# mschoenb97/po2_quantization

Measured on AMD Instinct MI355X. Metric: quantized-conv fwd images/sec, ResNet56 224×224 bs=256; 1/2/4/8 MI355X, higher is better.
Workload: dtype fp32(bf16x3); 1 GPU; resnet56 quantized-conv chain: 56 fused po2-4bit quantize+conv fwd + head (stage-1 and stage-2 conv1->conv2 pairs as one launch each) (stride-2 conv1 + 1x1 shortcut of stages 2-3 as one launch each) (weight packs of the single-conv layers batched: one launch per 36); conv_pairs=True, conv_pairs_stage2=True, s2ds=True, pack_batch=True, autotune=True, image=224, batch_per_gpu=256, global_batch=256, quantizer=po2, bits=4, precision=bf16x3, parallelism=dp1, world_size=1, hip_graph=False

## Files before the change

### po2_quantization_amd/csrc/po2q_capi.hip

```cpp
#include <hip/hip_runtime.h>

#include <cstdio>
#include <algorithm>
#include <new>
#include <cstring>
#include <string>
#include <vector>

#include "../../include/po2q.h"
#include "po2q_epi.h"
#include "po2q_internal.h"

namespace po2q {
static thread_local std::string g_last_error;
void set_error(const std::string& msg) { g_last_error = msg; }
}

using namespace po2q;

namespace {

constexpr size_t kAlign = 256;
size_t align_up(size_t v) { return (v + kAlign - 1) / kAlign * kAlign; }

// ... 875 lines not shown

int po2q_qconv2d_ir_f32(const float* x, float* y, const po2q_conv_plan* expand, const void* ws_e, size_t ws_e_bytes,
                        const po2q_conv_plan* depthwise, const void* ws_d, size_t ws_d_bytes,
                        const po2q_conv_plan* project, const void* ws_p, size_t ws_p_bytes, const float* ps1,
                        const float* pb1, int act1, const float* ps2, const float* pb2, int act2, const float* ps3,
                        const float* pb3, const float* residual, int act3, void* stream) {
    using namespace po2q;
    if (!x || !y || !ws_d || !ws_p || (expand && !ws_e)) {
        set_error("po2q: inverted residual: null pointer");
        return PO2Q_ERR_INVALID;
    }
    for (int a : {act1, act2, act3})
        if (a < PO2Q_ACT_NONE || a > PO2Q_ACT_SILU) {
            set_error("po2q: unknown activation " + std::to_string(a));
            return PO2Q_ERR_INVALID;
        }
    IrPlan ip;
    int64_t sh[7];
    int st = ir_check(expand, depthwise, project, &ip, sh);
    if (st) return st;
    const po2q_conv_plan* hs[3] = {expand, depthwise, project};
    const void* wss[3] = {ws_e, ws_d, ws_p};
    const size_t wsb[3] = {ws_e_bytes, ws_d_bytes, ws_p_bytes};
    const char* at[3] = {nullptr, nullptr, nullptr};
    const float* sc[3] = {nullptr, nullptr, nullptr};
    for (int i = 0; i < 3; ++i) {
        if (!hs[i]) continue;
        const WsLayout L = ws_layout(hs[i]->p, hs[i]->mode);
        if (wsb[i] < L.total) {
            set_error("po2q: inverted residual: workspace too small (need " + std::to_string(L.total) + " bytes)");
            return PO2Q_ERR_WORKSPACE;
        }
        at[i] = reinterpret_cast<const char*>(wss[i]) + L.packed_off;
        sc[i] = reinterpret_cast<const float*>(reinterpret_cast<const char*>(wss[i]) + L.scale_off);
    }
    const IrEpi ep{ps1, pb1, ps2, pb2, ps3, pb3, act1, act2, act3, residual};
    return hip_status(launch_conv_ir(ip, x, y, (int)sh[0], (int)sh[1], (int)sh[2], (int)sh[3], (int)sh[4], (int)sh[5],
                                     (int)sh[6], reinterpret_cast<const uint16_t*>(at[0]), sc[0],
                                     reinterpret_cast<const float*>(at[1]), reinterpret_cast<const uint16_t*>(at[2]),
                                     sc[2], ep, reinterpret_cast<hipStream_t>(stream)),
                      "inverted residual launch");
}

int po2q_qconv2d_plan_describe(const po2q_conv_plan* plan, char* buf, size_t len) {
    if (!plan || !buf || len == 0) {
        po2q::set_error("po2q: null plan or buffer");
        return PO2Q_ERR_INVALID;
    }
    describe_plan(plan->p, buf, len);
    return PO2Q_OK;
}

void po2q_qconv2d_plan_destroy(po2q_conv_plan* plan) { delete plan; }
```

### po2_quantization_amd/csrc/po2q_conv_chain.hip

```cpp
#include <hip/hip_runtime.h>

#include <algorithm>
#include <cstddef>
#include <cstdint>
#include <cstdlib>
#include <string>
#include <type_traits>
#include <utility>
#include <vector>

#include "../../include/po2q.h"
#ifdef PO2Q_CHAIN_STAMPS
#include <cstdio>
#endif
#include "po2q_epi.h"
#include "po2q_internal.h"
#include "po2q_x3_dev.h"

namespace po2q {

namespace {
constexpr int kChainThreads = 512;
constexpr int kChainItems = 5;
constexpr int kChainMax = PO2Q_CHAIN_MAX_LAYERS;
// ... 367 lines not shown
#endif
}

static int chain_mg(int64_t C, int64_t H, int64_t W) {
    const int64_t groups = (H * W + 15) / 16, wpt = (kChainThreads / 64) / (C / 16);
    return (int)((groups + wpt - 1) / wpt);
}
static int chain_mg_max(int64_t C) { return C == 16 ? 8 : 4; }

static bool chain_geom_ok(int64_t N, int64_t C, int64_t H, int64_t W, int n_layers) {
    if (!(C == 16 || C == 32 || C == 64) || N < 1 || H < 1 || W < 4 || W % 4 != 0) return false;
    if (n_layers < 1 || n_layers > kChainMax || N > INT32_MAX) return false;
    if (N * C * H * W >= (1LL << 40) || chain_mg(C, H, W) > chain_mg_max(C)) return false;
    return 3 * chain_plane(C, H, W) <= kChainLdsMax;
}

static bool chain_mode_ok(int bits, int fsr, int mode) {
    if (mode != PO2Q_MODE_PO2 && mode != PO2Q_MODE_PO2_PLUS) return false;
    if (bits < 1 || bits > 16) return false;
    const long lo = (long)fsr - (1L << (bits - 1)), hi = (long)fsr - 1;
    return lo >= -126 && hi <= 127;
}

static ConvPlan chain_plan(int64_t N, int64_t C, int64_t H, int64_t W) {
    ConvPlan p{};
    p.N = (int)N; p.C = (int)C; p.H = (int)H; p.W = (int)W; p.K = (int)C;
    p.R = p.S = 3; p.sh = p.sw = 1; p.ph = p.pw = 1; p.dh = p.dw = 1; p.groups = 1;
    p.P = p.H; p.Q = p.W; p.Cg = p.C; p.Kg = p.K;
    p.kind = KIND_BF16X3_IMG;
    p.CC = C == 16 ? 16 : 32;
    p.nchunks = (int)C / p.CC;
    p.steps = C == 16 ? 2 : 3 * p.nchunks;
    p.NT = (int)C / 16;
    p.taps = 9;
    p.packed_floats = (int64_t)3 * p.steps * p.NT * 64 * 4;
    return p;
}

namespace {
constexpr size_t kChainAlign = 256;
size_t chain_align(size_t v) { return (v + kChainAlign - 1) / kChainAlign * kChainAlign; }
struct ChainWs {
    size_t packed_off, packed_bytes, scale_off, total;
};
ChainWs chain_ws(int64_t N, int64_t C, int64_t H, int64_t W, int n_layers) {
    ChainWs L;
    const ConvPlan p = chain_plan(N, C, H, W);
    L.packed_bytes = chain_align((size_t)p.packed_floats * 4);
    L.packed_off = 0;
    L.scale_off = L.packed_bytes * (size_t)n_layers;
    L.total = L.scale_off + chain_align((size_t)n_layers * 4);
    return L;
}
}

}

using namespace po2q;

extern "C" {

int po2q_qconv2d_chain_supported(int64_t N, int64_t C, int64_t H, int64_t W, int n_layers, int bits, int fsr,
                                 int mode) {
    return chain_geom_ok(N, C, H, W, n_layers) && chain_mode_ok(bits, fsr, mode) ? 1 : 0;
}

size_t po2q_qconv2d_chain_workspace_bytes(int64_t N, int64_t C, int64_t H, int64_t W, int n_layers) {
    if (!chain_geom_ok(N, C, H, W, n_layers)) return 0;
    return chain_ws(N, C, H, W, n_layers).total;
}

int po2q_qconv2d_chain_f32(const float* x, const float* const* w, const float* const* bias,
                           const float* const* post_scale, const float* const* post_shift, const int* act,
                           const int* res_from, int n_layers, int64_t N, int64_t C, int64_t H, int64_t W, int bits,
                           int fsr, int mode, float* y, void* workspace, size_t workspace_bytes, void* stream) {
    if (po2q::is_lin_mode(mode)) {
        po2q::set_error("po2q: chain does not take the lin / lin+ modes");
        return PO2Q_ERR_UNSUPPORTED;
    }
    if (!chain_geom_ok(N, C, H, W, n_layers)) {
        set_error("po2q: chain needs C in {16, 32, 64}, W % 4 == 0, 1.." + std::to_string(kChainMax) +
                  " layers and a small image: its split planes in LDS ((H + 2)(W + 2) 6C bytes <= 160 KiB) and "
                  "at most 8 (C = 16) / 4 (C = 32, 64) 16-pixel groups per wave");
        return PO2Q_ERR_INVALID;
    }
    if (!chain_mode_ok(bits, fsr, mode)) {
        set_error("po2q: chain needs mode po2 / po2+ with exponents in the bf16 range");
        return PO2Q_ERR_INVALID;
    }
    if (!x || !w || !y || !workspace) {
        set_error("po2q: chain: null pointer");
        return PO2Q_ERR_INVALID;
    }
    const ChainWs L = chain_ws(N, C, H, W, n_layers);
    if (workspace_bytes < L.total) {
        set_error("po2q: chain workspace too small (need " + std::to_string(L.total) + " bytes)");
        return PO2Q_ERR_WORKSPACE;
    }
    for (int l = 0; l < n_layers; ++l) {
        if (!w[l]) {
            set_error("po2q: chain: null weight of layer " + std::to_string(l));
            return PO2Q_ERR_INVALID;
        }
        const int ac = act ? act[l] : 0;
        if (ac < 0 || ac > 3) {
            set_error("po2q: chain: unknown activation of layer " + std::to_string(l));
            return PO2Q_ERR_INVALID;
        }
        const int r = res_from ? res_from[l] : -1;
        if (r < -1 || r > l) {
            set_error("po2q: chain: res_from[" + std::to_string(l) + "] must be -1 or a layer index <= " +
                      std::to_string(l) + " (the residual is that layer's input)");
            return PO2Q_ERR_INVALID;
        }
    }
    for (int l1 = 0; l1 < n_layers; ++l1)
        for (int l2 = l1 + 1; l2 < n_layers; ++l2) {
            const int r1 = res_from ? res_from[l1] : -1, r2 = res_from ? res_from[l2] : -1;
            if (r1 >= 0 && r2 >= 0 && r1 != r2 && r2 <= l1) {
                set_error("po2q: chain: res_from holds one residual source at a time (layers " + std::to_string(l1) +
                          " and " + std::to_string(l2) + " add different, overlapping sources)");
                return PO2Q_ERR_INVALID;
            }
        }
    hipStream_t s = reinterpret_cast<hipStream_t>(stream);
    char* ws = reinterpret_cast<char*>(workspace);

    const ConvPlan plan = chain_plan(N, C, H, W);
    std::vector<const ConvPlan*> plans((size_t)n_layers, &plan);
    std::vector<uint16_t*> packed((size_t)n_layers);
    std::vector<float*> scales((size_t)n_layers);
    for (int l = 0; l < n_layers; ++l) {
        packed[l] = reinterpret_cast<uint16_t*>(ws + L.packed_off + (size_t)l * L.packed_bytes);
        scales[l] = reinterpret_cast<float*>(ws + L.scale_off) + l;
    }
    hipError_t he = launch_pack_bf16x3_batch(n_layers, plans.data(), w, packed.data(), scales.data(), bits, fsr,
                                             mode, s);
    if (he != hipSuccess) {
        set_error(std::string("po2q: chain weight pack launch: ") + hipGetErrorString(he));
        return PO2Q_ERR_HIP;
    }

    std::vector<int> used((size_t)n_layers + 1, 0);
    for (int l = 0; l < n_layers; ++l)
        if (res_from && res_from[l] >= 0) used[res_from[l]] = 1;
    ChainArgs a{};
    a.stamps = nullptr;
    a.H = (int)H; a.W = (int)W; a.L = n_layers;
    a.PW = (int)W + 2;
    a.PL = (int)chain_plane(C, H, W);
    a.ZO = a.PL - 16;
    a.res0 = used[0];
    for (int l = 0; l < n_layers; ++l) {
        ChainLayer& ly = a.layer[l];
        ly.wp = reinterpret_cast<const uint4*>(packed[l]);
        ly.scale = scales[l];
        ly.bias = bias ? bias[l] : nullptr;
        ly.ps = post_scale ? post_scale[l] : nullptr;
        ly.pb = post_shift ? post_shift[l] : nullptr;
        ly.act = act ? act[l] : 0;
        ly.res_add = (res_from && res_from[l] >= 0) ? 1 : 0;
        ly.keep = used[l + 1];
    }
    const char* venv = getenv("PO2Q_CHAIN_VARIANT");
    const int variant = venv ? atoi(venv) : 0;
    const bool db = !(variant & 8) && C != 16 && 6 * (size_t)a.PL <= kChainLdsMax;
    const size_t lds = (db ? 6 : 3) * (size_t)a.PL;
    const dim3 grid((unsigned)N), block(kChainThreads);
    const int mg = chain_mg(C, H, W);
    const bool w8 = C == 64 && W == 8;
    const int64_t wpt = (kChainThreads / 64) / (C / 16);
    const bool full = !(variant & 1) && (H * W) % 16 == 0 && (H * W / 16) % wpt == 0;
    auto launch = [&](const ChainArgs& a) -> bool {
#define PO2Q_CH(c, m, w)                                                                               \
    if (C == c && mg <= m && w8 == w) {                                                                \
        if (c != 16 && db) {                                                                           \
            if (full && mg == m)                                                                       \
                hipLaunchKernelGGL((conv_chain<c, m, w, true, true>), grid, block, lds, s, x, y, a);   \
            else                                                                                       \
// ... 52 lines not shown
```

### po2_quantization_amd/csrc/po2q_conv_pair.hip

```cpp
#include <hip/hip_runtime.h>

#include <algorithm>
#include <climits>
#include <cstdint>
#include <string>
#include <type_traits>
#ifdef PO2Q_PAIR_STAMPS
#include <cstdio>
#include <cstdlib>
#include <vector>
#endif

#include "../../include/po2q.h"
#include "po2q_epi.h"
#include "po2q_internal.h"
#include "po2q_quant_dev.h"
#include "po2q_rows_dev.h"
#include "po2q_x3_dev.h"

namespace po2q {

namespace {
template <int CC> constexpr int kQSW = 512 / CC;
template <int CC> constexpr int kQPlane = (kQSW<CC> + 2) * 2 * CC + 32;
// ... 1004 lines not shown
        return pp.pd == 3 ? launch_pair_rs<3>(pp, a, x, y, s) : hipErrorInvalidValue;
    }
#ifdef PO2Q_PAIR_DIAG
    if (const char* dv = getenv("PO2Q_PAIR_DEBUG")) {
        const int dbg = atoi(dv);
        const dim3 grid((unsigned)pp.blocks), block(64 * pp.waves);
#define PO2Q_PD(v) \
        if (dbg == v && pp.C == 16 && pp.pd == 2 && pp.nts == 3 && !res) { \
            hipLaunchKernelGGL((conv_pair<16, 2, 3, false, 0, v>), grid, block, pp.lds, s, x, y, a); \
            return hipGetLastError(); \
        }
        PO2Q_PD(1) PO2Q_PD(2) PO2Q_PD(3) PO2Q_PD(4) PO2Q_PD(8) PO2Q_PD(12) PO2Q_PD(16) PO2Q_PD(19)
        PO2Q_PD(15) PO2Q_PD(31)
#undef PO2Q_PD
    }
#endif
#define PO2Q_PR(c, d, nt) \
    if (pp.C == c && pp.pd == d && pp.nts == nt) return launch_pair_t<c, d, nt>(pp, a, x, y, res, s);
#ifdef PO2Q_PAIR_ISA_ONLY
    PO2Q_PR(16, 5, 3) PO2Q_PR(32, 2, 3)
    return hipErrorInvalidValue;
#endif
    PO2Q_PR(16, 2, 0) PO2Q_PR(16, 2, 1) PO2Q_PR(16, 2, 3) PO2Q_PR(32, 2, 0) PO2Q_PR(32, 2, 3)
    PO2Q_PR(16, 5, 3) PO2Q_PR(16, 6, 3)
#undef PO2Q_PR
    return hipErrorInvalidValue;
}

}

namespace {

void pair_variant(int& pd, int& nts, int& prio, int64_t C) {
    pd = 2;
    nts = 3;
    prio = C == 16 ? 1 : 0;
    if (const char* e = getenv("PO2Q_PAIR_VARIANT")) {
        const int v = atoi(e) % 1000;
        const int d = (v / 10) % 10, t = v % 10;
        prio = v >= 100 ? 1 : 0;
        if (d == 2 && (t == 0 || t == 3 || (t == 1 && C == 16))) {
            pd = d;
            nts = t;
        }
    }
}

bool pair_args_ok(int64_t N, int64_t C, int64_t H, int64_t W, int bits, int fsr, int mode, int act1, int act2) {
    if (N <= 0 || H <= 0 || W <= 0) {
        po2q::set_error("po2q: pair: sizes must be positive");
        return false;
    }
    if (C != 16 && C != 32) {
        po2q::set_error("po2q: pair: 16 or 32 channels only (ResNet56 stages 1 and 2)");
        return false;
    }
    if (mode != PO2Q_MODE_PO2 && mode != PO2Q_MODE_PO2_PLUS) {
        po2q::set_error("po2q: pair: mode must be po2 or po2+");
        return false;
    }
    if (bits < 1 || bits > 16) {
        po2q::set_error("po2q: bits must be in [1, 16]");
        return false;
    }
    const long lo = (long)fsr - (1L << (bits - 1)), hi = (long)fsr - 1;
    if (lo < -126 || hi > 127) {
        po2q::set_error("po2q: pair: the exponent window leaves the bf16 range");
        return false;
    }
    if (act1 < 0 || act1 > 3 || act2 < 0 || act2 > 3) {
        po2q::set_error("po2q: unknown activation");
        return false;
    }
    if (W % 4 != 0 || W > 7 * (512 / C)) {
        po2q::set_error("po2q: pair: W must be a multiple of 4 and at most 7 x 512 / C (224 for C = 16, 112 for 32)");
        return false;
    }
    return true;
}

}

int po2q_qconv2d_pair_supported(int64_t N, int64_t C, int64_t H, int64_t W, int bits, int fsr, int mode) {
    if ((C == 16 || C == 32) && W <= 3 * (512 / C)) return 0;
    if (C == 32) {
        const char* e = getenv("PO2Q_PAIR_C32");
        if (e && e[0] == '0') return 0;
    }
    po2q::PairPlan pp;
    int pd, nts, prio;
    pair_variant(pd, nts, prio, C);
    return pair_args_ok(N, C, H, W, bits, fsr, mode, 0, 0) &&
                   po2q::pair_plan(pp, (int)N, (int)C, (int)H, (int)W, true, pd, nts)
               ? 1
               : 0;
}

int po2q_qconv2d_pair_f32(const float* x, const float* w1, const float* w2, float* y, int64_t N, int64_t C,
                          int64_t H, int64_t W, int bits, int fsr, int mode, const float* bias1, const float* bias2,
                          const float* post_scale1, const float* post_shift1, int act1, const float* post_scale2,
                          const float* post_shift2, const float* residual, int act2, void* stream) {
    if (po2q::is_lin_mode(mode)) {
        po2q::set_error("po2q: pair does not take the lin / lin+ modes");
        return PO2Q_ERR_UNSUPPORTED;
    }
    if (!pair_args_ok(N, C, H, W, bits, fsr, mode, act1, act2)) return PO2Q_ERR_INVALID;
    if (!x || !w1 || !w2 || !y) {
        po2q::set_error("po2q: null pointer");
        return PO2Q_ERR_INVALID;
    }
    if (residual == y || x == y) {
        po2q::set_error("po2q: pair: y must not alias x or the residual");
        return PO2Q_ERR_INVALID;
    }
    if (po2q::pairw_applicable(N, C, H, W)) {
        const hipError_t e = po2q::pairw_launch(x, w1, w2, y, N, H, W, bits, fsr, mode, bias1, bias2, post_scale1,
                                                post_shift1, act1, post_scale2, post_shift2, residual, act2,
                                                reinterpret_cast<hipStream_t>(stream));
        if (e != hipSuccess) {
            po2q::set_error(std::string("po2q: pair launch: ") + hipGetErrorString(e));
            return PO2Q_ERR_HIP;
        }
        return PO2Q_OK;
    }
    po2q::PairPlan pp;
    int pd, nts, prio;
    pair_variant(pd, nts, prio, C);
    if (residual && C == 16 && !getenv("PO2Q_PAIR_VARIANT")) {
        pd = 2;
        nts = 1;
        prio = 0;
    }
    if (!po2q::pair_plan(pp, (int)N, (int)C, (int)H, (int)W, residual != nullptr, pd, nts)) {
        po2q::set_error("po2q: pair: no plan for this shape");
        return PO2Q_ERR_UNSUPPORTED;
    }
    po2q::PairArgs a;
    a.N = (int)N; a.H = (int)H; a.W = (int)W;
    a.Wp = (512 / (int)C) * pp.waves;
    a.YPL = (7 * (512 / (int)C) + 3) * 2 * (int)C;
    a.RB = pp.RB; a.nseg = pp.nseg; a.items = (int)(N * pp.nseg);
    a.remap = (pp.blocks % 8 == 0) ? 1 : 0;
    const int lo = fsr - (1 << (bits - 1)), hi = fsr - 1;
    a.q1.w = w1; a.q1.n = (int)(C * C * 9); a.q1.lo = lo; a.q1.hi = hi; a.q1.mode = mode - 1;
    a.q2 = a.q1;
    a.q2.w = w2;
    a.b1 = bias1; a.b2 = bias2;
    a.ps1 = post_scale1; a.pb1 = post_shift1; a.act1 = act1;
    a.ps2 = post_scale2; a.pb2 = post_shift2; a.act2 = act2;
    a.res = residual;
    a.prio = prio;
    a.stamps = nullptr;
    a.mw = 0;
    {
        const char* rsv = getenv("PO2Q_PAIR_RS");
        const bool rs_on = rsv ? rsv[0] != '0' : (!getenv("PO2Q_PAIR_MW") && !getenv("PO2Q_PAIR_VARIANT"));
        const int d = 3;
// ... 38 lines not shown
```

### po2_quantization_amd/csrc/po2q_internal.h

```cpp
#pragma once
#include <hip/hip_runtime.h>

#include <cstddef>
#include <cstdint>
#include <string>
#include <vector>

namespace po2q {

void set_error(const std::string& msg);

constexpr int kThreads = 256;
constexpr int kMaxPartials = 1024;
constexpr int64_t kFusedAbsmaxMax = 1 << 20;

int absmax_blocks(int64_t n);

hipError_t launch_absmax(const float* w, int64_t n, unsigned* partial, int blocks, hipStream_t s);

hipError_t launch_quantize_plain(const float* w, int64_t n, const unsigned* partial, int nparts,
                                 int bits, int fsr, int mode, float* out, hipStream_t s);

inline bool is_lin_mode(int mode) { return mode == 3 || mode == 4; }
inline bool lin_bf16x3_ok(int bits, int num_iters, int groups) {
// ... 110 lines not shown
    void* packed;
    float* scale;
    int bits, fsr, mode;
    unsigned* partial = nullptr;
    const float* delta = nullptr;
};
bool pack_batchable(const ConvPlan& p, int mode);
hipError_t launch_pack_batch(int n, const PackReq* reqs, hipStream_t s);
hipError_t launch_pack_bf16x3_batch(int n, const ConvPlan* const* plans, const float* const* w,
                                    uint16_t* const* packed, float* const* scale_out, int bits, int fsr, int mode,
                                    hipStream_t s);

bool dw3_plan(ConvPlan& p);
bool dw3_plan_ok(const ConvPlan& p);
hipError_t launch_conv_dw3(const ConvPlan& p, const float* x, const float* qw, const float* bias, float* y,
                           const float* ps, const float* pb, const float* res, int act, hipStream_t s);
hipError_t launch_conv(const ConvPlan& p, const float* x, const float* packed, const float* bias,
                       float* y, hipStream_t s);

hipError_t launch_conv_bf16x3(const ConvPlan& p, const float* x, const uint16_t* packed,
                              const float* scale, const float* bias, float* y, hipStream_t s);

hipError_t launch_conv_bf16x3_rows(const ConvPlan& p, const float* x, const uint16_t* packed,
                                   const float* scale, const float* bias, float* y, hipStream_t s,
                                   const WQuant& q = WQuant{});

hipError_t launch_conv_bf16x3_dma(const ConvPlan& p, const float* x, const uint16_t* packed,
                                  const float* scale, const float* bias, float* y, hipStream_t s);

struct IrPlan {
    int G, R, RI, nbands, CHK, P, PG, Po, HP, xs;
    size_t lds, off_hid, off_dpl, off_cw;
    int64_t blocks;
    int small = 0;
    int ntw = 0, tg = 0;
};
struct IrEpi {
    const float *ps1, *pb1, *ps2, *pb2, *ps3, *pb3;
    int act1, act2, act3;
    const float* res;
};
bool ir_plan(IrPlan& ip, int64_t N, int64_t Cin, int64_t H, int64_t W, int64_t Ch, int64_t Cout, int64_t S,
             bool expand);
hipError_t launch_conv_ir(const IrPlan& ip, const float* x, float* y, int N, int Cin, int H, int W, int Ch, int Cout,
                          int S, const uint16_t* we, const float* we_scale, const float* wd, const uint16_t* wp,
                          const float* wp_scale, const IrEpi& e, hipStream_t s);

bool pairw_applicable(int64_t N, int64_t C, int64_t H, int64_t W);
hipError_t pairw_launch(const float* x, const float* w1, const float* w2, float* y, int64_t N, int64_t H,
                        int64_t W, int bits, int fsr, int mode, const float* bias1, const float* bias2,
                        const float* post_scale1, const float* post_shift1, int act1, const float* post_scale2,
                        const float* post_shift2, const float* residual, int act2, hipStream_t s);

template <typename T>
hipError_t launch_quantize_dt(const T* w, T* out, int64_t n, int bits, int fsr, int mode, uint64_t* partial,
                              int nparts, hipStream_t s);

struct B16Epi {
    const float* ps = nullptr;
    const float* pb = nullptr;
    const uint16_t* res = nullptr;
    int act = 0;
    bool any() const { return ps || pb || res || act != 0; }
};
int b16_plan(ConvPlan& p);
size_t b16_workspace_bytes(const ConvPlan& p);
void b16_describe(const ConvPlan& p, char* buf, size_t len);
hipError_t b16_run(const ConvPlan& p, const uint16_t* x, const uint16_t* w, const uint16_t* bias, uint16_t* y,
                   int bits, int fsr, int mode, void* workspace, hipStream_t s, const B16Epi& e = B16Epi{});
struct B16PackReq {
    const ConvPlan* plan;
    const uint16_t* w;
    void* workspace;
    int bits, fsr, mode;
};
hipError_t b16_pack_batch(int n, const B16PackReq* reqs, hipStream_t s);
hipError_t b16_run_packed(const ConvPlan& p, const uint16_t* x, const uint16_t* bias, uint16_t* y,
                          const void* workspace, hipStream_t s, const B16Epi& e = B16Epi{});

hipError_t launch_quantize_lin(const float* w, float* out, int d0, int d1, int rs, int bits, int num_iters, int plus,
                               hipStream_t s);
struct LinReq {
    const float* w;
    float* delta;
    int d0, d1, rs, bits, num_iters, plus;
};
hipError_t launch_lin_delta_batch(int n, const LinReq* reqs, hipStream_t s);

}
```

Baseline: 26040 images/s.

## Add 64-channel conv-pair kernel and chain path for stage-3 sized images

```diff
diff --git a/po2_quantization_amd/csrc/po2q_capi.hip b/po2_quantization_amd/csrc/po2q_capi.hip
--- a/po2_quantization_amd/csrc/po2q_capi.hip
+++ b/po2_quantization_amd/csrc/po2q_capi.hip
@@ -951,3 +951,30 @@
 }
 
 void po2q_qconv2d_plan_destroy(po2q_conv_plan* plan) { delete plan; }
+
+namespace po2q {
+
+bool single_plan(ConvPlan& p, int64_t N, int64_t C, int64_t H, int64_t W, int bits, int fsr, int mode) {
+    return make_plan(p, N, C, H, W, C, 3, 3, 1, 1, 1, 1, 1, 1, 1, mode, bits, fsr, PO2Q_PREC_AUTO);
+}
+
+SingleWs single_ws(const ConvPlan& p, int mode) {
+    const WsLayout L = ws_layout(p, mode);
+    SingleWs w;
+    w.total = L.total;
+    w.scale_off = L.scale_off;
+    w.packed_off = L.packed_off;
+    w.batch = plan_packs_weight(p, mode) && is_bf16x3_kind(p.kind) && pack_batchable(p, mode) && L.nparts == 0;
+    return w;
+}
+
+size_t single_ws_max(int64_t N, int64_t C, int64_t H, int64_t W) {
+    return po2q_qconv2d_workspace_bytes(N, C, H, W, C, 3, 3, 1, 1, 1, 1, 1, 1, 1, 4, 1, PO2Q_MODE_PO2, PO2Q_PREC_AUTO);
+}
+
+int single_run(const ConvPlan& p, const float* x, const float* w, const float* bias, float* y, int bits, int fsr,
+               int mode, void* workspace, size_t workspace_bytes, hipStream_t s, const ConvEpi& e, bool packed) {
+    return run_plan(p, x, w, bias, y, bits, fsr, mode, workspace, workspace_bytes, s, e, packed ? RUN_CONV : RUN_ALL);
+}
+
+}
diff --git a/po2_quantization_amd/csrc/po2q_conv_chain.hip b/po2_quantization_amd/csrc/po2q_conv_chain.hip
--- a/po2_quantization_amd/csrc/po2q_conv_chain.hip
+++ b/po2_quantization_amd/csrc/po2q_conv_chain.hip
@@ -443,6 +443,123 @@
     L.total = L.scale_off + chain_align((size_t)n_layers * 4);
     return L;
 }
+
+bool chain64_geom_ok(int64_t N, int64_t C, int64_t H, int64_t W, int n_layers) {
+    return pair64_enabled() && pair64_geom_ok(N, C, H, W) && n_layers >= 2 && n_layers <= kChainMax;
+}
+
+struct Chain64Ws {
+    size_t slot, act_off, act_bytes, total;
+};
+Chain64Ws chain64_ws(int64_t N, int64_t C, int64_t H, int64_t W, int n_layers) {
+    Chain64Ws L;
+    L.slot = chain_align(std::max(kChainAlign + pair64_pack_bytes(), single_ws_max(N, C, H, W)));
+    L.act_off = L.slot * (size_t)n_layers;
+    L.act_bytes = chain_align((size_t)(N * C * H * W) * 4);
+    L.total = L.act_off + 2 * L.act_bytes;
+    return L;
+}
+
+struct Chain64Launch {
+    int l0, len;
+    int out;
+};
+
+bool chain64_assign(std::vector<Chain64Launch>& ls, size_t k, std::vector<int>& buf, const int* res_from, int n) {
+    if (k == ls.size()) return true;
+    Chain64Launch& c = ls[k];
+    const bool last = k + 1 == ls.size();
+    for (int b = last ? 2 : 0; b < 3; ++b) {
+        bool ok = buf[c.l0] != b;
+        for (int l = c.l0; ok && l < n; ++l) {
+            const int r = res_from ? res_from[l] : -1;
+            if (r >= 0 && r <= c.l0 && buf[r] == b) ok = false;
+        }
+        if (!ok) continue;
+        c.out = b;
+        buf[c.l0 + c.len] = b;
+        if (chain64_assign(ls, k + 1, buf, res_from, n)) return true;
+    }
+    return false;
+}
+
+int chain64_run(const float* x, const float* const* w, const float* const* bias, const float* const* post_scale,
+                const float* const* post_shift, const int* act, const int* res_from, int n, int64_t N, int64_t C,
+                int64_t H, int64_t W, int bits, int fsr, int mode, float* y, char* ws, hipStream_t s) {
+    const Chain64Ws L = chain64_ws(N, C, H, W, n);
+    ConvPlan sp;
+    if (!single_plan(sp, N, C, H, W, bits, fsr, mode)) return PO2Q_ERR_INVALID;
+    const SingleWs sw = single_ws(sp, mode);
+    if (sw.total > L.slot) {
+        set_error("po2q: chain: the single-conv plan's workspace exceeds the layer slot");
+        return PO2Q_ERR_WORKSPACE;
+    }
+    std::vector<int> used((size_t)n + 1, 0);
+    for (int l = 0; l < n; ++l)
+        if (res_from && res_from[l] >= 0) used[res_from[l]] = 1;
+    auto plain = [&](int l) {
+        return !(post_scale && post_scale[l]) && !(post_shift && post_shift[l]) && !(act && act[l] != 0) &&
+               !(res_from && res_from[l] >= 0);
+    };
+    std::vector<Chain64Launch> ls;
+    for (int l = 0; l < n;) {
+        const bool pair = l + 1 < n && plain(l) && plain(l + 1) && !used[l + 1];
+        ls.push_back(Chain64Launch{l, pair ? 2 : 1, 2});
+        l += pair ? 2 : 1;
+    }
+    std::vector<int> buf((size_t)n + 1, -2);
+    buf[0] = -1;
+    if (!chain64_assign(ls, 0, buf, res_from, n)) {
+        set_error("po2q: chain: no activation buffer rotation for this res_from pattern");
+        return PO2Q_ERR_INVALID;
+    }
+    auto slot = [&](int l) { return ws + (size_t)l * L.slot; };
+    auto bufp = [&](int b) -> float* {
+        return b == 2 ? y : reinterpret_cast<float*>(ws + L.act_off + (size_t)b * L.act_bytes);
+    };
+    auto actp = [&](int j) -> const float* { return j == 0 ? x : bufp(buf[j]); };
+
+    const ConvPlan pk = pair64_pack_plan(N, H, W);
+    std::vector<PackReq> reqs;
+    for (const Chain64Launch& c : ls)
+        for (int l = c.l0; l < c.l0 + c.len; ++l) {
+            if (c.len == 2)
+                reqs.push_back(PackReq{&pk, w[l], slot(l) + kChainAlign, reinterpret_cast<float*>(slot(l)), bits, fsr, mode});
+            else if (sw.batch)
+                reqs.push_back(PackReq{&sp, w[l], slot(l) + sw.packed_off, reinterpret_cast<float*>(slot(l) + sw.scale_off),
+                                       bits, fsr, mode});
+        }
+    if (!reqs.empty()) {
+        const hipError_t he = launch_pack_batch((int)reqs.size(), reqs.data(), s);
+        if (he != hipSuccess) {
+            set_error(std::string("po2q: chain weight pack launch: ") + hipGetErrorString(he));
+            return PO2Q_ERR_HIP;
+        }
+    }
+    for (const Chain64Launch& c : ls) {
+        const int l = c.l0;
+        const float* in = actp(l);
+        float* out = bufp(c.out);
+        if (c.len == 2) {
+            const hipError_t he = pair64_launch(
+                in, out, N, H, W, reinterpret_cast<const uint16_t*>(slot(l) + kChainAlign),
+                reinterpret_cast<const float*>(slot(l)), reinterpret_cast<const uint16_t*>(slot(l + 1) + kChainAlign),
+                reinterpret_cast<const float*>(slot(l + 1)), bias ? bias[l] : nullptr, bias ? bias[l + 1] : nullptr, s);
+            if (he != hipSuccess) {
+                set_error(std::string("po2q: chain pair launch: ") + hipGetErrorString(he));
+                return PO2Q_ERR_HIP;
+            }
+            continue;
+        }
+        const int r = res_from ? res_from[l] : -1;
+        const ConvEpi e{post_scale ? post_scale[l] : nullptr, post_shift ? post_shift[l] : nullptr,
+                        r >= 0 ? actp(r) : nullptr, act ? act[l] : 0};
+        const int st = single_run(sp, in, w[l], bias ? bias[l] : nullptr, out, bits, fsr, mode, slot(l), L.slot, s, e,
+                                  sw.batch);
+        if (st) return st;
+    }
+    return PO2Q_OK;
+}
 }
 
 }
@@ -453,12 +570,16 @@
 
 int po2q_qconv2d_chain_supported(int64_t N, int64_t C, int64_t H, int64_t W, int n_layers, int bits, int fsr,
                                  int mode) {
-    return chain_geom_ok(N, C, H, W, n_layers) && chain_mode_ok(bits, fsr, mode) ? 1 : 0;
+    return (chain_geom_ok(N, C, H, W, n_layers) || chain64_geom_ok(N, C, H, W, n_layers)) &&
+                   chain_mode_ok(bits, fsr, mode)
+               ? 1
+               : 0;
 }
 
 size_t po2q_qconv2d_chain_workspace_bytes(int64_t N, int64_t C, int64_t H, int64_t W, int n_layers) {
-    if (!chain_geom_ok(N, C, H, W, n_layers)) return 0;
-    return chain_ws(N, C, H, W, n_layers).total;
+    if (chain_geom_ok(N, C, H, W, n_layers)) return chain_ws(N, C, H, W, n_layers).total;
+    if (chain64_geom_ok(N, C, H, W, n_layers)) return chain64_ws(N, C, H, W, n_layers).total;
+    return 0;
 }
 
 int po2q_qconv2d_chain_f32(const float* x, const float* const* w, const float* const* bias,
@@ -469,10 +590,12 @@
         po2q::set_error("po2q: chain does not take the lin / lin+ modes");
         return PO2Q_ERR_UNSUPPORTED;
     }
-    if (!chain_geom_ok(N, C, H, W, n_layers)) {
+    const bool big = !chain_geom_ok(N, C, H, W, n_layers) && chain64_geom_ok(N, C, H, W, n_layers);
+    if (!big && !chain_geom_ok(N, C, H, W, n_layers)) {
         set_error("po2q: chain needs C in {16, 32, 64}, W % 4 == 0, 1.." + std::to_string(kChainMax) +
-                  " layers and a small image: its split planes in LDS ((H + 2)(W + 2) 6C bytes <= 160 KiB) and "
-                  "at most 8 (C = 16) / 4 (C = 32, 64) 16-pixel groups per wave");
+                  " layers and either a small image (one launch): its split planes in LDS ((H + 2)(W + 2) 6C bytes "
+                  "<= 160 KiB) and at most 8 (C = 16) / 4 (C = 32, 64) 16-pixel groups per wave; or C = 64 with "
+                  "32 < W <= 64 and at least 2 layers (a run of conv-pair launches; PO2Q_PAIR64=0 turns it off)");
         return PO2Q_ERR_INVALID;
     }
     if (!chain_mode_ok(bits, fsr, mode)) {
@@ -483,9 +606,10 @@
         set_error("po2q: chain: null pointer");
         return PO2Q_ERR_INVALID;
     }
-    const ChainWs L = chain_ws(N, C, H, W, n_layers);
-    if (workspace_bytes < L.total) {
-        set_error("po2q: chain workspace too small (need " + std::to_string(L.total) + " bytes)");
+    const ChainWs L = big ? ChainWs{} : chain_ws(N, C, H, W, n_layers);
+    const size_t need = big ? chain64_ws(N, C, H, W, n_layers).total : L.total;
+    if (workspace_bytes < need) {
+        set_error("po2q: chain workspace too small (need " + std::to_string(need) + " bytes)");
         return PO2Q_ERR_WORKSPACE;
     }
     for (int l = 0; l < n_layers; ++l) {
@@ -516,6 +640,14 @@
         }
     hipStream_t s = reinterpret_cast<hipStream_t>(stream);
     char* ws = reinterpret_cast<char*>(workspace);
+    if (big) {
+        if (x == y) {
+            set_error("po2q: chain: y must not alias x");
+            return PO2Q_ERR_INVALID;
+        }
+        return chain64_run(x, w, bias, post_scale, post_shift, act, res_from, n_layers, N, C, H, W, bits, fsr, mode, y,
+                           ws, s);
+    }
 
     const ConvPlan plan = chain_plan(N, C, H, W);
     std::vector<const ConvPlan*> plans((size_t)n_layers, &plan);
diff --git a/po2_quantization_amd/csrc/po2q_conv_pair.hip b/po2_quantization_amd/csrc/po2q_conv_pair.hip
--- a/po2_quantization_amd/csrc/po2q_conv_pair.hip
+++ b/po2_quantization_amd/csrc/po2q_conv_pair.hip
@@ -1080,7 +1080,7 @@
         return false;
     }
     if (C != 16 && C != 32) {
-        po2q::set_error("po2q: pair: 16 or 32 channels only (ResNet56 stages 1 and 2)");
+        po2q::set_error("po2q: pair: 16 or 32 channels only (ResNet56 stages 1 and 2), or 64 with 32 < W <= 64");
         return false;
     }
     if (mode != PO2Q_MODE_PO2 && mode != PO2Q_MODE_PO2_PLUS) {
@@ -1131,6 +1131,11 @@
     if (po2q::is_lin_mode(mode)) {
         po2q::set_error("po2q: pair does not take the lin / lin+ modes");
         return PO2Q_ERR_UNSUPPORTED;
+    }
+    if (C == 64 && po2q::pair64_geom_ok(N, C, H, W)) {
+        const bool plain = !post_scale1 && !post_shift1 && !post_scale2 && !post_shift2 && !residual && act1 == 0 &&
+                           act2 == 0;
+        return po2q::pair64_entry(x, w1, w2, y, N, H, W, bits, fsr, mode, bias1, bias2, plain, stream);
     }
     if (!pair_args_ok(N, C, H, W, bits, fsr, mode, act1, act2)) return PO2Q_ERR_INVALID;
     if (!x || !w1 || !w2 || !y) {
diff --git a/po2_quantization_amd/csrc/po2q_conv_pair64.hip b/po2_quantization_amd/csrc/po2q_conv_pair64.hip
--- /dev/null
+++ b/po2_quantization_amd/csrc/po2q_conv_pair64.hip
@@ -0,0 +1,439 @@
+#include <hip/hip_runtime.h>
+
+#include <algorithm>
+#include <climits>
+#include <cstdint>
+#include <cstdlib>
+#include <map>
+#include <mutex>
+#include <string>
+#include <type_traits>
+#include <utility>
+
+#include "../../include/po2q.h"
+#include "po2q_internal.h"
+#include "po2q_rows_dev.h"
+#include "po2q_x3_dev.h"
+
+namespace po2q {
+
+namespace {
+constexpr int kP6C = 64;
+constexpr int kP6Wp = 64;
+constexpr int kP6PL = (kP6Wp + 2) * 2 * kP6C;
+constexpr int kP6Set = 3 * kP6PL;
+constexpr int kP6Raw = kP6C * kP6Wp * 4;
+constexpr int kP6RPB = kP6Wp * 4;
+constexpr int kP6PD = 2;
+constexpr int kP6KS = 6;
+constexpr int kP6Lds = kP6PD * kP6Raw + 2 * kP6Set + 2 * kP6Set;
+constexpr int kP6PackBytes = 3 * kP6KS * 4 * 64 * 16;
+
+__device__ __forceinline__ int p6_addr(int P, int oc) { return P * 128 + ((oc ^ (P & 7)) << 4); }
+}
+
+struct Pair64Args {
+    int N, H, W;
+    int RB, nseg, items, remap;
+    const uint4* wp1;
+    const uint4* wp2;
+    const float* s1;
+    const float* s2;
+    const float* b1;
+    const float* b2;
+};
+
+template <int NG, int NTS>
+__global__ __launch_bounds__(512, 1) void conv_pair64(const float* __restrict__ x, float* __restrict__ y,
+                                                      Pair64Args a) {
+    static_assert(NG == 3 || NG == 4, "column groups");
+    constexpr int C = kP6C, KS = kP6KS, PL = kP6PL, SET = kP6Set, RPB = kP6RPB;
+    extern __shared__ __attribute__((aligned(16))) unsigned char lds[];
+    const int tid = threadIdx.x, lane = tid & 63;
+    const int wave = __builtin_amdgcn_readfirstlane(tid >> 6);
+    const bool roleA = wave >= 4;
+    const int t = wave & 3;
+    unsigned char* raw = lds;
+    unsigned char* xp = raw + kP6PD * kP6Raw;
+
+    int blk = blockIdx.x;
+    if (a.remap) blk = (blk & 7) * (int)(gridDim.x >> 3) + (blk >> 3);
+    if (blk >= a.items) return;
+    const int seg = blk % a.nseg;
+    const int n = blk / a.nseg;
+    const int p0 = seg * a.RB;
+    const int rbe = min(a.RB, a.H - p0);
+    const int nx = rbe + 4;
+    const int n1 = rbe + 2;
+    const int nsteps = nx + 2;
+    const int HW = a.H * a.W;
+
+    bf16x8 bw[3][KS];
+    {
+        const uint4* wp = roleA ? a.wp2 : a.wp1;
+#pragma unroll
+        for (int r = 0; r < 3; ++r)
+#pragma unroll
+            for (int ks = 0; ks < KS; ++ks) bw[r][ks] = __builtin_bit_cast(bf16x8, wp[((r * KS + ks) * 4 + t) * 64 + lane]);
+    }
+    float scale = *(roleA ? a.s2 : a.s1);
+    float bk[4];
+    {
+        const float* b = roleA ? a.b2 : a.b1;
+#pragma unroll
+        for (int e = 0; e < 4; ++e) bk[e] = b ? b[roleA ? 16 * t + (lane & 15) : 16 * t + 4 * (lane >> 4) + e] : 0.0f;
+    }
+#pragma unroll
+    for (int r = 0; r < 3; ++r)
+#pragma unroll
+        for (int ks = 0; ks < KS; ++ks) asm volatile("s_waitcnt vmcnt(0)" : "+v"(bw[r][ks]));
+    asm volatile("s_waitcnt vmcnt(0)" : "+v"(scale), "+v"(bk[0]), "+v"(bk[1]), "+v"(bk[2]), "+v"(bk[3]));
+
+    for (int e = tid; e < (4 * SET) / 16; e += 512) reinterpret_cast<uint4*>(xp)[e] = make_uint4(0u, 0u, 0u, 0u);
+    __syncthreads();
+
+    const __amdgpu_buffer_rsrc_t rs = rows_rsrc(x + (int64_t)n * C * HW, C * HW * 4);
+    uint32_t vi[4];
+#pragma unroll
+    for (int i = 0; i < 4; ++i) {
+        const int c = 16 * t + 4 * i + (lane >> 4), q = 4 * (lane & 15);
+        vi[i] = q < a.W ? ((uint32_t)c * (uint32_t)HW + (uint32_t)q) * 4u : 0x7fffffffu;
+    }
+    const uint32_t raw_lds = (uint32_t)(uintptr_t)raw;
+    auto load_x = [&](int sl, int jn) __attribute__((always_inline)) {
+        const int h = p0 - 2 + jn;
+        const bool hok = jn < nx && h >= 0 && h < a.H;
+        const uint32_t roff = (uint32_t)(hok ? h : 0) * (uint32_t)a.W * 4u;
+        const uint32_t base = raw_lds + (uint32_t)(sl * kP6Raw) + (uint32_t)(16 * t) * (uint32_t)RPB;
+#pragma unroll
+        for (int i = 0; i < 4; ++i)
+            rows_dma16<(NTS & 2) != 0>(rs, (hok && vi[i] != 0x7fffffffu) ? vi[i] + roff : 0x7fffffffu, 0u,
+                                       base + (uint32_t)i * 1024u);
+    };
+    int xwb[2] = {p6_addr(lane + 1, 2 * t) + kP6PD * kP6Raw, p6_addr(lane + 1, 2 * t + 1) + kP6PD * kP6Raw};
+    asm volatile("" : "+v"(xwb[0]), "+v"(xwb[1]));
+    auto split_x = [&](const unsigned char* rw, int pb) __attribute__((always_inline)) {
+#pragma unroll
+        for (int o = 0; o < 2; ++o) {
+            uint32_t b8[8];
+#pragma unroll
+            for (int e = 0; e < 8; ++e)
+                b8[e] = *reinterpret_cast<const uint32_t*>(rw + (16 * t + 8 * o + e) * RPB + lane * 4);
+            uint4 hi, mid, lo;
+            split3(b8, hi, mid, lo);
+            unsigned char* pw = lds + (xwb[o] + pb);
+            *reinterpret_cast<uint4*>(pw) = hi;
+            *reinterpret_cast<uint4*>(pw + PL) = mid;
+            *reinterpret_cast<uint4*>(pw + 2 * PL) = lo;
+        }
+    };
+
+    int foff[KS];
+    {
+        const int p = lane & 15, g = lane >> 4;
+        const int region = kP6PD * kP6Raw + (roleA ? 2 * SET : 0);
+#pragma unroll
+        for (int ks = 0; ks < KS; ++ks) {
+            foff[ks] = p6_addr(p + ks % 3, 4 * (ks / 3) + g) + region;
+            asm volatile("" : "+v"(foff[ks]));
+        }
+    }
+    int ywb = p6_addr((lane & 15) + 1, 2 * t + (lane >> 5)) + 8 * ((lane >> 4) & 1) + kP6PD * kP6Raw + 2 * SET;
+    asm volatile("" : "+v"(ywb));
+
+    floatx4 acc[3][NG];
+#pragma unroll
+    for (int sl = 0; sl < 3; ++sl)
+#pragma unroll
+        for (int grp = 0; grp < NG; ++grp) acc[sl][grp] = floatx4{0.f, 0.f, 0.f, 0.f};
+
+    auto mfmas = [&](auto S_, auto TR_, int pb) __attribute__((always_inline)) {
+        constexpr int S = decltype(S_)::value;
+        constexpr bool TR = decltype(TR_)::value;
+        constexpr int SL[3] = {(S + 1) % 3, S, (S + 2) % 3};
+        bf16x8 af[2][NG];
+        auto ldf = [&](bf16x8 (&f)[NG], int st) __attribute__((always_inline)) {
+#pragma unroll
+            for (int grp = 0; grp < NG; ++grp)
+                f[grp] = __builtin_bit_cast(
+                    bf16x8, *reinterpret_cast<const uint4*>(lds + (foff[st / 3] + (pb + (st % 3) * PL + grp * (16 * 128)))));
+        };
+        ldf(af[0], 0);
+#pragma unroll
+        for (int st = 0; st < 3 * KS; ++st) {
+            if (st + 1 < 3 * KS) ldf(af[(st + 1) & 1], st + 1);
+            const int ks = st / 3;
+#pragma unroll
+            for (int rr = 0; rr < 3; ++rr)
+#pragma unroll
+                for (int grp = 0; grp < NG; ++grp)
+                    acc[SL[rr]][grp] =
+                        TR ? __builtin_amdgcn_mfma_f32_16x16x32_bf16(bw[rr][ks], af[st & 1][grp], acc[SL[rr]][grp], 0, 0, 0)
+                           : __builtin_amdgcn_mfma_f32_16x16x32_bf16(af[st & 1][grp], bw[rr][ks], acc[SL[rr]][grp], 0, 0, 0);
+            __builtin_amdgcn_sched_barrier(0);
+        }
+    };
+
+    floatx4 pend[NG];
+#pragma unroll
+    for (int grp = 0; grp < NG; ++grp) pend[grp] = floatx4{0.f, 0.f, 0.f, 0.f};
+
+    auto stepB = [&](auto S_, int j) __attribute__((always_inline)) {
+        constexpr int S6 = decltype(S_)::value;
+        constexpr int S = S6 % 3;
+        constexpr int D = (S + 2) % 3;
+        constexpr int B2 = S6 & 1;
+        asm volatile("s_waitcnt lgkmcnt(0)\n\ts_barrier" ::: "memory");
+        load_x(B2, j + 2);
+        {
+            const int i1 = j - 3;
+            const int r1 = p0 - 1 + i1;
+            const bool irow = i1 >= 0 && i1 < n1 && r1 >= 0 && r1 < a.H;
+            const int p = lane & 15;
+            unsigned char* yw = lds + (ywb + (1 - B2) * SET);
+#pragma unroll
+            for (int grp = 0; grp < NG; ++grp) {
+                const int q = 16 * grp + p;
+                const bool okq = irow && q < a.W;
+                uint32_t b4[4];
+#pragma unroll
+                for (int e = 0; e < 4; ++e) {
+                    const float v = pend[grp][e] * scale + bk[e];
+                    b4[e] = okq ? __float_as_uint(v) : 0u;
+                }
+                uint2 h2, m2, l2;
+                split4p(b4, h2, m2, l2);
+                unsigned char* yg = yw + grp * (16 * 128);
+                *reinterpret_cast<uint2*>(yg) = h2;
+                *reinterpret_cast<uint2*>(yg + PL) = m2;
+                *reinterpret_cast<uint2*>(yg + 2 * PL) = l2;
+            }
+        }
+        rows_wait<4>();
+        split_x(raw + (1 - B2) * kP6Raw, (1 - B2) * SET);
+        {
+            const int h = p0 - 2 + j;
+            if (j < nx && h >= 0 && h < a.H) mfmas(std::integral_constant<int, S>{}, std::true_type{}, B2 * SET);
+        }
+#pragma unroll
+        for (int grp = 0; grp < NG; ++grp) {
+            pend[grp] = acc[D][grp];
+            acc[D][grp] = floatx4{0.f, 0.f, 0.f, 0.f};
+        }
+    };
+
+    const __amdgpu_buffer_rsrc_t ry = rows_rsrc(y + (int64_t)n * C * HW, C * HW * 4);
+
+    auto stepA = [&](auto S_, int j) __attribute__((always_inline)) {
+        constexpr int S6 = decltype(S_)::value;
+        constexpr int S = S6 % 3;
+        constexpr int D = (S + 2) % 3;
+        constexpr int YR = S6 & 1;
+        asm volatile("s_waitcnt lgkmcnt(0)\n\ts_barrier" ::: "memory");
+        {
+            const int i2 = j - 4, r2 = p0 - 1 + i2;
+            if (i2 >= 0 && i2 < n1 && r2 >= 0 && r2 < a.H)
+                mfmas(std::integral_constant<int, S>{}, std::false_type{}, YR * SET);
+        }
+        const int o = j - 6;
+        const bool orow = o >= 0 && o < rbe;
+        const int g = lane >> 4;
+        const uint32_t ca = (uint32_t)(16 * t) + (uint32_t)(lane & 7), cb = ca + 8u;
+#pragma unroll
+        for (int pr = 0; pr < 2; ++pr) {
+            floatx4 vv[2];
+#pragma unroll
+            for (int h = 0; h < 2; ++h) {
+                const int grp = 2 * pr + h;
+                if (grp < NG) {
+#pragma unroll
+                    for (int e = 0; e < 4; ++e) vv[h][e] = acc[D][grp][e] * scale + bk[0];
+                    acc[D][grp] = floatx4{0.f, 0.f, 0.f, 0.f};
+                } else {
+                    vv[h] = floatx4{0.f, 0.f, 0.f, 0.f};
+                }
+            }
+            floatx4 sa, sb;
+#pragma unroll
+            for (int e = 0; e < 4; ++e) {
+                sa[e] = __int_as_float(__builtin_amdgcn_update_dpp(__float_as_int(vv[0][e]), __float_as_int(vv[1][e]),
+                                                                   0x128, 0xf, 0xc, false));
+                sb[e] = __int_as_float(__builtin_amdgcn_update_dpp(__float_as_int(vv[1][e]), __float_as_int(vv[0][e]),
+                                                                   0x128, 0xf, 0x3, false));
+            }
+            const int qs = 32 * pr + ((lane & 8) ? 16 : 0) + 4 * g;
+            const bool ok = orow && qs < a.W;
+            const uint32_t rowoff = (uint32_t)(orow ? p0 + o : 0) * (uint32_t)a.W + (uint32_t)qs;
+            rows_store<(NTS & 1) != 0>(ry, ok ? (ca * (uint32_t)HW + rowoff) * 4u : 0x7fffffffu, sa);
+            rows_store<(NTS & 1) != 0>(ry, ok ? (cb * (uint32_t)HW + rowoff) * 4u : 0x7fffffffu, sb);
+        }
+    };
+
+    if (roleA) {
+        for (int j = 0; j < nsteps; j += 6) {
+            stepA(std::integral_constant<int, 0>{}, j);
+            stepA(std::integral_constant<int, 1>{}, j + 1);
+            stepA(std::integral_constant<int, 2>{}, j + 2);
+            if (j + 3 >= nsteps) break;
+            stepA(std::integral_constant<int, 3>{}, j + 3);
+            stepA(std::integral_constant<int, 4>{}, j + 4);
+            stepA(std::integral_constant<int, 5>{}, j + 5);
+        }
+    } else {
+        load_x(0, 0);
+        load_x(1, 1);
+        rows_wait<4>();
+        split_x(raw, 0);
+        for (int j = 0; j < nsteps; j += 6) {
+            stepB(std::integral_constant<int, 0>{}, j);
+            stepB(std::integral_constant<int, 1>{}, j + 1);
+            stepB(std::integral_constant<int, 2>{}, j + 2);
+            if (j + 3 >= nsteps) break;
+            stepB(std::integral_constant<int, 3>{}, j + 3);
+            stepB(std::integral_constant<int, 4>{}, j + 4);
+            stepB(std::integral_constant<int, 5>{}, j + 5);
+        }
+    }
+    asm volatile("s_waitcnt vmcnt(0)" ::: "memory");
+}
+
+bool pair64_enabled() {
+    const char* e = getenv("PO2Q_PAIR64");
+    return !(e && e[0] == '0');
+}
+
+bool pair64_geom_ok(int64_t N, int64_t C, int64_t H, int64_t W) {
+    return C == kP6C && W > 32 && W <= kP6Wp && W % 4 == 0 && N > 0 && H > 0 && C * H * W * 4 < (1LL << 31) &&
+           N * H <= INT_MAX / 2;
+}
+
+size_t pair64_pack_bytes() { return (size_t)kP6PackBytes; }
+
+hipError_t pair64_launch(const float* x, float* y, int64_t N, int64_t H, int64_t W, const uint16_t* packed1,
+                         const float* scale1, const uint16_t* packed2, const float* scale2, const float* bias1,
+                         const float* bias2, hipStream_t s) {
+    if (!pair64_geom_ok(N, kP6C, H, W)) return hipErrorInvalidValue;
+    int64_t nseg = std::max<int64_t>(1, (256 + N - 1) / N);
+    nseg = std::min<int64_t>(nseg, std::max<int64_t>(1, H / 8));
+    if (const char* e = getenv("PO2Q_PAIR64_NSEG")) nseg = std::min<int64_t>(std::max(1, atoi(e)), H);
+    Pair64Args a;
+    a.N = (int)N; a.H = (int)H; a.W = (int)W;
+    a.RB = (int)((H + nseg - 1) / nseg);
+    a.nseg = (int)((H + a.RB - 1) / a.RB);
+    const int64_t items = N * a.nseg;
+    if (items > INT_MAX / 2) return hipErrorInvalidValue;
+    const int blocks = (int)((items + 7) / 8 * 8);
+    a.items = (int)items;
+    a.remap = 1;
+    a.wp1 = reinterpret_cast<const uint4*>(packed1);
+    a.wp2 = reinterpret_cast<const uint4*>(packed2);
+    a.s1 = scale1; a.s2 = scale2;
+    a.b1 = bias1; a.b2 = bias2;
+    int nts = 0;
+    if (const char* e = getenv("PO2Q_PAIR64_NTS")) nts = atoi(e) == 0 ? 0 : 3;
+    const dim3 grid((unsigned)blocks), block(512);
+#define PO2Q_P6(g, t)                                                                            \
+    if ((W <= 48 ? 3 : 4) == g && nts == t) {                                                    \
+        hipLaunchKernelGGL((conv_pair64<g, t>), grid, block, (size_t)kP6Lds, s, x, y, a);        \
+        return hipGetLastError();                                                                \
+    }
+    PO2Q_P6(4, 3) PO2Q_P6(3, 3) PO2Q_P6(4, 0) PO2Q_P6(3, 0)
+#undef PO2Q_P6
+    return hipErrorInvalidValue;
+}
+
+ConvPlan pair64_pack_plan(int64_t N, int64_t H, int64_t W) {
+    ConvPlan p{};
+    p.N = (int)N; p.C = kP6C; p.H = (int)H; p.W = (int)W; p.K = kP6C;
+    p.R = p.S = 3; p.sh = p.sw = 1; p.ph = p.pw = 1; p.dh = p.dw = 1; p.groups = 1;
+    p.P = p.H; p.Q = p.W; p.Cg = p.C; p.Kg = p.K;
+    p.kind = KIND_BF16X3_ROWS;
+    p.vrx = 1;
+    p.CC = 32;
+    p.nchunks = 2;
+    p.steps = kP6KS;
+    p.NT = 4;
+    p.taps = 9;
+    p.packed_floats = kP6PackBytes / 4;
+    return p;
+}
+
+namespace {
+constexpr size_t kP6Scratch = 256 + 2 * ((kP6PackBytes + 255) / 256 * 256);
+char* pair64_scratch(hipStream_t s) {
+    static std::mutex mu;
+    static std::map<std::pair<int, hipStream_t>, char*> pool;
+    int dev = 0;
+    if (hipGetDevice(&dev) != hipSuccess) return nullptr;
+    std::lock_guard<std::mutex> lock(mu);
+    auto it = pool.find({dev, s});
+    if (it != pool.end()) return it->second;
+    void* p = nullptr;
+    if (hipMalloc(&p, kP6Scratch) != hipSuccess) {
+        (void)hipGetLastError();
+        return nullptr;
+    }
+    pool[{dev, s}] = reinterpret_cast<char*>(p);
+    return reinterpret_cast<char*>(p);
+}
+}
+
+int pair64_entry(const float* x, const float* w1, const float* w2, float* y, int64_t N, int64_t H, int64_t W,
+                 int bits, int fsr, int mode, const float* bias1, const float* bias2, bool plain, void* stream) {
+    if (mode != PO2Q_MODE_PO2 && mode != PO2Q_MODE_PO2_PLUS) {
+        set_error("po2q: pair: mode must be po2 or po2+");
+        return PO2Q_ERR_INVALID;
+    }
+    if (bits < 1 || bits > 16) {
+        set_error("po2q: bits must be in [1, 16]");
+        return PO2Q_ERR_INVALID;
+    }
+    const long lo = (long)fsr - (1L << (bits - 1)), hi = (long)fsr - 1;
+    if (lo < -126 || hi > 127) {
+        set_error("po2q: pair: the exponent window leaves the bf16 range");
+        return PO2Q_ERR_INVALID;
+    }
+    if (!pair64_geom_ok(N, kP6C, H, W)) {
+        set_error("po2q: pair: 64 channels take 32 < W <= 64 with W % 4 == 0 (ResNet56 stage 3 at 56 x 56)");
+        return PO2Q_ERR_INVALID;
+    }
+    if (!plain) {
+        set_error("po2q: pair: 64 channels take the plain form only (biases; no BN affine, activation or residual): "
+                  "run the two layers with po2q_qconv2d_fused_f32");
+        return PO2Q_ERR_UNSUPPORTED;
+    }
+    if (!x || !w1 || !w2 || !y) {
+        set_error("po2q: null pointer");
+        return PO2Q_ERR_INVALID;
+    }
+    if (x == y) {
+        set_error("po2q: pair: y must not alias x or the residual");
+        return PO2Q_ERR_INVALID;
+    }
+    hipStream_t s = reinterpret_cast<hipStream_t>(stream);
+    char* ws = pair64_scratch(s);
+    if (!ws) {
+        set_error("po2q: pair: no device memory for the weight packs (the first 64-channel call on a stream "
+                  "allocates them: make it outside a graph capture)");
+        return PO2Q_ERR_HIP;
+    }
+    const ConvPlan plan = pair64_pack_plan(N, H, W);
+    const size_t pb = (kP6PackBytes + 255) / 256 * 256;
+    const ConvPlan* plans[2] = {&plan, &plan};
+    const float* ws_[2] = {w1, w2};
+    uint16_t* packed[2] = {reinterpret_cast<uint16_t*>(ws + 256), reinterpret_cast<uint16_t*>(ws + 256 + pb)};
+    float* scales[2] = {reinterpret_cast<float*>(ws), reinterpret_cast<float*>(ws) + 1};
+    hipError_t he = launch_pack_bf16x3_batch(2, plans, ws_, packed, scales, bits, fsr, mode, s);
+    if (he != hipSuccess) {
+        set_error(std::string("po2q: pair weight pack launch: ") + hipGetErrorString(he));
+        return PO2Q_ERR_HIP;
+    }
+    he = pair64_launch(x, y, N, H, W, packed[0], scales[0], packed[1], scales[1], bias1, bias2, s);
+    if (he != hipSuccess) {
+        set_error(std::string("po2q: pair launch: ") + hipGetErrorString(he));
+        return PO2Q_ERR_HIP;
+    }
+    return PO2Q_OK;
+}
+
+}
diff --git a/po2_quantization_amd/csrc/po2q_internal.h b/po2_quantization_amd/csrc/po2q_internal.h
--- a/po2_quantization_amd/csrc/po2q_internal.h
+++ b/po2_quantization_amd/csrc/po2q_internal.h
@@ -186,6 +186,27 @@
                         const float* post_scale1, const float* post_shift1, int act1, const float* post_scale2,
                         const float* post_shift2, const float* residual, int act2, hipStream_t s);
 
+bool pair64_enabled();
+bool pair64_geom_ok(int64_t N, int64_t C, int64_t H, int64_t W);
+size_t pair64_pack_bytes();
+ConvPlan pair64_pack_plan(int64_t N, int64_t H, int64_t W);
+hipError_t pair64_launch(const float* x, float* y, int64_t N, int64_t H, int64_t W, const uint16_t* packed1,
+                         const float* scale1, const uint16_t* packed2, const float* scale2, const float* bias1,
+                         const float* bias2, hipStream_t s);
+int pair64_entry(const float* x, const float* w1, const float* w2, float* y, int64_t N, int64_t H, int64_t W,
+                 int bits, int fsr, int mode, const float* bias1, const float* bias2, bool plain, void* stream);
+
+struct SingleWs {
+    size_t total, scale_off, packed_off;
+    bool batch;
+};
+bool single_plan(ConvPlan& p, int64_t N, int64_t C, int64_t H, int64_t W, int bits, int fsr, int mode);
+SingleWs single_ws(const ConvPlan& p, int mode);
+size_t single_ws_max(int64_t N, int64_t C, int64_t H, int64_t W);
+struct ConvEpi;
+int single_run(const ConvPlan& p, const float* x, const float* w, const float* bias, float* y, int bits, int fsr,
+               int mode, void* workspace, size_t workspace_bytes, hipStream_t s, const ConvEpi& e, bool packed);
+
 template <typename T>
 hipError_t launch_quantize_dt(const T* w, T* out, int64_t n, int bits, int fsr, int mode, uint64_t* partial,
                               int nparts, hipStream_t s);
```

Result: faster. 26700 images/s, median of 6 (+2.5%).
